# google-deepmind/dqn_zoo

Measured on NVIDIA H100. Metric: learner_grad_steps_per_sec, higher is better.
Workload: dtype f32 (f64 sum tree)

## Files before the change

### dqn_zoo_b200/csrc/dz_async.cuh

```cuda
#pragma once
#include <cuda_runtime.h>
#include <stdint.h>

namespace dz {

__device__ __forceinline__ uint32_t smem_u32(const void* p) { return (uint32_t)__cvta_generic_to_shared(p); }

__device__ __forceinline__ uint32_t smem_pad_1024(const void* base) {
  const uint32_t addr = smem_u32(base);
  return ((addr + 1023u) & ~1023u) - addr;
}

__device__ __forceinline__ void mbar_init(uint64_t* bar, uint32_t count) {
  asm volatile("mbarrier.init.shared::cta.b64 [%0], %1;" ::"r"(smem_u32(bar)), "r"(count));
}
__device__ __forceinline__ void fence_mbarrier_init() { asm volatile("fence.mbarrier_init.release.cluster;" ::: "memory"); }
__device__ __forceinline__ void mbar_arrive(uint64_t* bar) {
  asm volatile("mbarrier.arrive.shared::cta.b64 _, [%0];" ::"r"(smem_u32(bar)) : "memory");
}
__device__ __forceinline__ void mbar_arrive_if(uint64_t* bar, bool pred) {
  asm volatile("{\n.reg .pred p;\nsetp.ne.b32 p, %1, 0;\n@p mbarrier.arrive.shared::cta.b64 _, [%0];\n}\n" ::"r"(smem_u32(bar)),
               "r"((int)pred)
               : "memory");
}
// ... 13 lines not shown
      "r"(parity)
      : "memory");
}

__device__ __forceinline__ bool elect_one() {
  uint32_t pred;
  asm volatile("{\n .reg .pred P;\n elect.sync _|P, 0xffffffff;\n selp.u32 %0, 1, 0, P;\n}\n" : "=r"(pred));
  return pred != 0;
}

__device__ __forceinline__ void bulk_g2s(uint32_t dst_smem, const void* src, uint32_t bytes, uint64_t* bar) {
  asm volatile("cp.async.bulk.shared::cluster.global.mbarrier::complete_tx::bytes [%0], [%1], %2, [%3];" ::"r"(dst_smem),
               "l"(__cvta_generic_to_global(src)), "r"(bytes), "r"(smem_u32(bar))
               : "memory");
}
__device__ __forceinline__ void bulk_s2g(void* dst, const void* src_smem, uint32_t bytes) {
  asm volatile("cp.async.bulk.global.shared::cta.bulk_group [%0], [%1], %2;" ::"l"(__cvta_generic_to_global(dst)),
               "r"(smem_u32(src_smem)), "r"(bytes)
               : "memory");
}
__device__ __forceinline__ void bulk_commit_group() { asm volatile("cp.async.bulk.commit_group;" ::: "memory"); }
__device__ __forceinline__ void bulk_wait_group() { asm volatile("cp.async.bulk.wait_group 0;" ::: "memory"); }
__device__ __forceinline__ void bulk_wait_group_read() { asm volatile("cp.async.bulk.wait_group.read 0;" ::: "memory"); }

__device__ __forceinline__ void tma_load_5d(uint32_t dst_smem, const void* map, uint64_t* bar, int c0, int c1, int c2, int c3, int c4) {
  asm volatile(
      "cp.async.bulk.tensor.5d.shared::cluster.global.mbarrier::complete_tx::bytes [%0], [%1, {%3, %4, %5, %6, %7}], [%2];" ::"r"(dst_smem),
      "l"(reinterpret_cast<uint64_t>(map)), "r"(smem_u32(bar)), "r"(c0), "r"(c1), "r"(c2), "r"(c3), "r"(c4)
      : "memory");
}
__device__ __forceinline__ void prefetch_tensormap(const void* map) {
  asm volatile("prefetch.tensormap [%0];" ::"l"(reinterpret_cast<uint64_t>(map)) : "memory");
}
// ... 5 lines not shown
```

### dqn_zoo_b200/csrc/dz_gemm.cuh

```cuda
#pragma once
#include "dz_common.cuh"

namespace dz {

enum : int { A_PLAIN = 0, A_CONV_F32 = 1, A_CONV_U8 = 2 };

struct FastDiv {
  uint32_t mul, shr;
  int d;
};
inline FastDiv make_fastdiv(int d) {
  FastDiv f;
  f.d = d < 1 ? 1 : d;
  uint32_t s = 0;
  while ((1u << s) < (uint32_t)f.d) ++s;
  f.shr = s;
  f.mul = (uint32_t)((((uint64_t)1 << 32) * (((uint64_t)1 << s) - (uint64_t)f.d)) / (uint64_t)f.d + 1);
  return f;
}
__device__ __forceinline__ int fd_div(int n, const FastDiv& f) {
  return (int)(((uint32_t)__umulhi((uint32_t)n, f.mul) + (uint32_t)n) >> f.shr);
}


// ... 9 lines not shown
  int H, W, Cin, KW, S, OH, OW, seg;
  FastDiv fd_per, fd_ow, fd_seg;
  const float* bias;
  const float* bias2;
  const float* a_scale;
  const float* c_scale;
  const float* mul;
  const float* mask;
  float* Cb;
  float* Cb2;
  int mul_div;
  int relu;
  int bias_shared;
  int splits;
  long long split_stride;
};

constexpr int kMaxProblems = 6;
struct GemmBatch {
  GemmProblem p[kMaxProblems];
  int n;
};

struct ARow {
  const float* f;
  const uint8_t* u;
};

__device__ __forceinline__ ARow a_row_base(const GemmProblem& p, int m) {
  ARow r{nullptr, nullptr};
// ... 350 lines not shown
      if (p.relu) v = fmaxf(v, 0.f);
      p.C[(long long)m * p.ldc + n] = v;
    }
  }
}

template <int BMK, int BN, int BR, int TM, int TN>
__global__ void __launch_bounds__((BMK / TM) * (BN / TN)) gemm_tn_kernel(const __grid_constant__ GemmBatch batch) {
  dz::pdl_enter();
  constexpr int NT = (BMK / TM) * (BN / TN);
  const GemmProblem& p = batch.p[blockIdx.z];
  const int Kext = p.K + ((p.Cb || p.Cb2) ? 1 : 0);
  const int tiles_k = (Kext + BMK - 1) / BMK;
  const int tile_k = blockIdx.y % tiles_k, split = blockIdx.y / tiles_k;
  const int kk0 = tile_k * BMK, n0 = blockIdx.x * BN;
  if (blockIdx.y >= tiles_k * p.splits || n0 >= p.N) return;
  const int rchunks = (p.M + BR - 1) / BR;
  const int per = (rchunks + p.splits - 1) / p.splits;
  const int rc0 = split * per, rc1 = min(rchunks, rc0 + per);

  __shared__ __align__(16) float As[2][BR][BMK + kPad];
  __shared__ __align__(16) float Bs[2][BR][BN + kPad];
  const int tid = threadIdx.x, tx = tid % (BN / TN), ty = tid / (BN / TN);
  constexpr int A_VEC = BR * BMK / 4, B_VEC = BR * BN / 4;
  constexpr int A_PER = (A_VEC + NT - 1) / NT, B_PER = (B_VEC + NT - 1) / NT;
  const bool vecG = (p.ldb % 4 == 0) && ((reinterpret_cast<uintptr_t>(p.B) & 15) == 0);
  Acc<TM, TN> acc;
  acc.clear();
  float4 ra[A_PER], rb[B_PER];
  auto gload = [&](int rc) {
    const int r0 = rc * BR;
// ... 37 lines not shown
      int v = tid + i * NT;
      if (v < B_VEC) *reinterpret_cast<float4*>(&Bs[buf][v / (BN / 4)][(v % (BN / 4)) * 4]) = rb[i];
    }
  };
  if (rc0 < rc1) { gload(rc0); sstore(0); }
  __syncthreads();
  for (int rc = rc0; rc < rc1; ++rc) {
    const int cur = (rc - rc0) & 1;
    const bool more = rc + 1 < rc1;
    if (more) gload(rc + 1);
    tile_fma<BMK, BN, BR, TM, TN, kPad>(As[cur], Bs[cur], ty, tx, acc);
    if (more) sstore(cur ^ 1);
    __syncthreads();
  }

#pragma unroll
  for (int i = 0; i < TM; ++i) {
    int k = kk0 + ty * TM + i;
    if (k >= Kext) continue;
    const int nb = n0 + tx * TN;
    if (TN == 4 && nb + 3 < p.N && (p.N % 4 == 0) && (p.ldc % 4 == 0 || p.split_stride > 0)) {
      float4 v4 = make_float4(acc.v[i][0], acc.v[i][1], acc.v[i][2], acc.v[i][3]);
      if (p.split_stride > 0) {
        *reinterpret_cast<float4*>(p.C + (long long)split * p.split_stride + (long long)k * p.N + nb) = v4;
        continue;
      }
      if (k < p.K) {
        if (p.C) *reinterpret_cast<float4*>(p.C + (long long)k * p.ldc + nb) = v4;
        if (p.C2) {
          float a = p.a_scale[k];
          float4 c = *reinterpret_cast<const float4*>(p.c_scale + nb);
          *reinterpret_cast<float4*>(p.C2 + (long long)k * p.ldc + nb) = make_float4(v4.x * a * c.x, v4.y * a * c.y, v4.z * a * c.z, v4.w * a * c.w);
        }
      } else {
        if (p.Cb) *reinterpret_cast<float4*>(p.Cb + nb) = v4;
        if (p.Cb2) {
          float4 c = *reinterpret_cast<const float4*>(p.c_scale + nb);
          *reinterpret_cast<float4*>(p.Cb2 + nb) = make_float4(v4.x * c.x, v4.y * c.y, v4.z * c.z, v4.w * c.w);
        }
      }
      continue;
    }
#pragma unroll
    for (int j = 0; j < TN; ++j) {
      int n = n0 + tx * TN + j;
      if (n >= p.N) continue;
      float v = acc.v[i][j];
      if (p.split_stride > 0) {
        p.C[(long long)split * p.split_stride + (long long)k * p.N + n] = v;
        continue;
      }
      if (k < p.K) {
        if (p.C) p.C[(long long)k * p.ldc + n] = v;
        if (p.C2) p.C2[(long long)k * p.ldc + n] = v * p.a_scale[k] * p.c_scale[n];
      } else {
        if (p.Cb) p.Cb[n] = v;
        if (p.Cb2) p.Cb2[n] = v * p.c_scale[n];
      }
    }
  }
}

template <int BM, int BNK, int BR, int TM, int TN, bool DUAL>
__global__ void __launch_bounds__((BM / TM) * (BNK / TN)) gemm_nt_kernel(const __grid_constant__ GemmBatch batch) {
  dz::pdl_enter();
  constexpr int NT = (BM / TM) * (BNK / TN);
  const GemmProblem& p = batch.p[blockIdx.z];
  const int tiles_m = (p.M + BM - 1) / BM;
  const int tile_m = blockIdx.y % tiles_m, split = blockIdx.y / tiles_m;
  const int m0 = tile_m * BM, k0 = blockIdx.x * BNK;
  if (blockIdx.y >= tiles_m * p.splits || k0 >= p.K) return;
  const int nchunks = (p.N + BR - 1) / BR;
  const int per = (nchunks + p.splits - 1) / p.splits;
// ... 99 lines not shown
```

### dqn_zoo_b200/csrc/dz_learner.cu

```cuda
#include <algorithm>
#include <cmath>
#include <map>
#include <vector>

#include "dz_async.cuh"
#include "dz_gemm.cuh"
#include "dz_tc.cuh"
#include "dz_internal.cuh"
#include "dz_umma_net.cuh"

namespace dz {


struct TensorInfo {
  std::string name;
  int64_t shape[4];
  int ndim;
  int64_t offset, count;
};

struct Dims {
  int H, W, C;
  int h1, w1, h2, w2, h3, w3;
  int feat;
// ... 292 lines not shown
        int oy = yy / S;
        if (oy >= OH) continue;
        for (int kw = 0; kw < KW; ++kw) {
          int xx = x - kw;
          if (xx < 0 || xx % S) continue;
          int ox = xx / S;
          if (ox >= OW) continue;
          v += dcol[((long long)(b * OH + oy) * OW + ox) * K + (kh * KW + kw) * Cin + c];
        }
      }
    }
    dx[i] = v;
  }
}

__global__ void sum_to_scalar_kernel(const float* __restrict__ v, int n, float* out) {
  dz::pdl_enter();
  __shared__ float s[32];
  float acc = 0.f;
  for (int i = threadIdx.x; i < n; i += blockDim.x) acc += v[i];
  acc = warp_sum(acc);
  if ((threadIdx.x & 31) == 0) s[threadIdx.x >> 5] = acc;
  __syncthreads();
  if (threadIdx.x < 32) {
    acc = threadIdx.x < (blockDim.x >> 5) ? s[threadIdx.x] : 0.f;
    acc = warp_sum(acc);
    if (threadIdx.x == 0) out[0] = acc;
  }
}


constexpr int kSkinnyMaxN = 18;
struct SkinnyHead { const float* A[3]; const float* W[3]; const float* bias[3]; float* out[3]; int M[3]; int n; };

__global__ void __launch_bounds__(256) iqn_head_fwd_kernel(const __grid_constant__ SkinnyHead h, int N) {
  dz::pdl_enter();
  constexpr int K = 512;
  __shared__ __align__(16) float Ws[kSkinnyMaxN * K];
  const int q = blockIdx.y;
  const float* __restrict__ W = h.W[q];
  for (int i = threadIdx.x; i < K * N; i += 256) {
    int k = i / N, n = i - k * N;
// ... 488 lines not shown
      res = e / s;
    } else if (kind == DZ_QRDQN || kind == DZ_IQN) {
      float s = 0.f;
      for (int j = tid; j < nq; j += blockDim.x) s += out[(long long)j * A + a];
      res = block_sum(s, red) / (float)nq;
    } else {
      res = out[a];
    }
    if (tid == 0) q[a] = res;
    __syncthreads();
  }
}


__global__ void __launch_bounds__(256) grad_norm_kernel(const float* __restrict__ g, long long n, float* partials,
                                                        unsigned int* ticket, float* norm_out, int64_t* counters, float* user_norm,
                                                        int sumsq_only) {
  dz::pdl_enter();
  __shared__ float s[32];
  __shared__ bool last;
  float acc = 0.f;
  const long long n4 = n >> 2;
  const float4* g4 = reinterpret_cast<const float4*>(g);
  for (long long i = blockIdx.x * (long long)blockDim.x + threadIdx.x; i < n4; i += (long long)gridDim.x * blockDim.x) {
    float4 v = g4[i];
    acc = fmaf(v.x, v.x, acc); acc = fmaf(v.y, v.y, acc); acc = fmaf(v.z, v.z, acc); acc = fmaf(v.w, v.w, acc);
  }
  acc = warp_sum(acc);
  if ((threadIdx.x & 31) == 0) s[threadIdx.x >> 5] = acc;
  __syncthreads();
  if (threadIdx.x == 0) {
    float t = 0.f;
// ... 3 lines not shown
    unsigned int done = atomicAdd(ticket, 1u);
    last = (done == gridDim.x - 1);
  }
  __syncthreads();
  if (last) {
    __threadfence();
    float t = 0.f;
    for (unsigned int i = threadIdx.x; i < gridDim.x; i += blockDim.x) t += ((volatile float*)partials)[i];
    t = warp_sum(t);
    __syncthreads();
    if ((threadIdx.x & 31) == 0) s[threadIdx.x >> 5] = t;
    __syncthreads();
    if (threadIdx.x == 0) {
      float tot = 0.f;
      for (int i = 0; i < (blockDim.x >> 5); ++i) tot += s[i];
      norm_out[0] = sumsq_only ? tot : sqrtf(tot);
      if (user_norm && !sumsq_only) user_norm[0] = norm_out[0];
      *ticket = 0;
      counters[0] += 1;
    }
  }
}

struct OptArgs {
  int kind; float lr, eps, decay, b1, b2, max_norm;
  float* p; const float* g; float* m; float* v; long long n; const float* norm; const int64_t* counters;
  const float* parts; int nparts; const float* fc_sumsq; float* norm_out; float* user_norm;
  int stages;
};

__device__ __forceinline__ float split_norm(const float* __restrict__ parts, int nparts, const float* __restrict__ fc_sumsq) {
  __shared__ float s_red[8];
  float t = 0.f;
  if (threadIdx.x < 256) {
    for (int i = threadIdx.x; i < nparts; i += 256) t += __ldcg(parts + i);
    t = warp_sum(t);
    if ((threadIdx.x & 31) == 0) s_red[threadIdx.x >> 5] = t;
  }
  __syncthreads();
  float tot = __ldcg(fc_sumsq);
#pragma unroll
  for (int i = 0; i < 8; ++i) tot += s_red[i];
  return sqrtf(tot);
}

__global__ void __launch_bounds__(256) norm_finalize_kernel(const float* parts, int nparts, const float* fc_sumsq, float* norm_out,
                                                            float* user_norm) {
  dz::pdl_enter();
  const float norm = split_norm(parts, nparts, fc_sumsq);
  if (threadIdx.x == 0) { norm_out[0] = norm; if (user_norm) user_norm[0] = norm; }
}

template <int KIND>
__device__ __forceinline__ float opt_one(const OptArgs& o, float p, float g, float& m, float& v, bool clip, float norm,
                                         float inv_c1, float inv_c2) {
  if (clip) g = (g / norm) * o.max_norm;
  float upd;
  if (KIND == DZ_ADAM) {
    float mu = o.b1 * m + (1.0f - o.b1) * g;
    float nu = o.b2 * v + (1.0f - o.b2) * g * g;
    if (fabsf(mu) < 1.17549435e-38f) mu = 0.f;
    if (nu < 1.17549435e-38f) nu = 0.f;
    m = mu; v = nu;
    upd = (mu * inv_c1) / (sqrtf(nu * inv_c2) + o.eps);
  } else {
// ... 20 lines not shown
  const int kOptStages = o.stages;
  uint64_t* full = reinterpret_cast<uint64_t*>(opt_sm + kOptStages * kOptStageBytes);
  const int tid = threadIdx.x;
  const long long n4 = o.n >> 2;
  const long long nchunks = (n4 + kOptChunk - 1) / kOptChunk;
  const long long mine = blockIdx.x < nchunks ? (nchunks - blockIdx.x + gridDim.x - 1) / gridDim.x : 0;
  float4* p4 = reinterpret_cast<float4*>(o.p);
  const float4* g4 = reinterpret_cast<const float4*>(o.g);
  float4* m4 = reinterpret_cast<float4*>(o.m);
  float4* v4 = reinterpret_cast<float4*>(o.v);
  if (tid == 0) {
    for (int s = 0; s < kOptStages; ++s) mbar_init(&full[s], 1);
    fence_mbarrier_init();
  }
  __syncthreads();
  dz::pdl_enter();
  auto issue = [&](long long it, int s) {
    const long long c = blockIdx.x + it * gridDim.x;
    const long long q0 = c * kOptChunk;
    const uint32_t bytes = (uint32_t)(min((long long)kOptChunk, n4 - q0) * 16);
    const uint32_t st = smem_u32(opt_sm + s * kOptStageBytes);
    mbar_expect_tx(&full[s], 4 * bytes);
    bulk_g2s(st, p4 + q0, bytes, &full[s]);
    bulk_g2s(st + kOptChunk * 16, g4 + q0, bytes, &full[s]);
    bulk_g2s(st + 2 * kOptChunk * 16, m4 + q0, bytes, &full[s]);
    bulk_g2s(st + 3 * kOptChunk * 16, v4 + q0, bytes, &full[s]);
  };
  if (tid == 0)
    for (long long it = 0; it < mine && it < kOptStages; ++it) issue(it, (int)it);
  float norm;
  if (o.parts != nullptr) {
    norm = split_norm(o.parts, o.nparts, o.fc_sumsq);
    if (blockIdx.x == 0 && tid == 0) { o.norm_out[0] = norm; if (o.user_norm) o.user_norm[0] = norm; }
  } else {
    norm = o.norm[0];
  }
  const bool clip = o.max_norm > 0.f && !(norm < o.max_norm);
  float c1 = 1.f, c2 = 1.f;
  if (KIND == DZ_ADAM) {
    float t = (float)o.counters[0];
    c1 = 1.0f / (1.0f - powf(o.b1, t));
    c2 = 1.0f / (1.0f - powf(o.b2, t));
  }
  int s = 0;
  uint32_t phase = 0;
  for (long long it = 0; it < mine; ++it) {
    const long long q0 = (blockIdx.x + it * gridDim.x) * (long long)kOptChunk;
    const int valid = (int)min((long long)kOptChunk, n4 - q0);
    float4* sp = reinterpret_cast<float4*>(opt_sm + s * kOptStageBytes);
    float4* sg = sp + kOptChunk;
    float4* smm = sp + 2 * kOptChunk;
    float4* sv = sp + 3 * kOptChunk;
    if (tid == 0 && it > 0) {
      const long long next = it - 1 + kOptStages;
      if (next < mine) {
        bulk_wait_group_read();
        issue(next, s == 0 ? kOptStages - 1 : s - 1);
      }
    }
    mbar_wait(&full[s], phase);
    if (tid < 2 * valid) {
      float2 p = reinterpret_cast<float2*>(sp)[tid], g = reinterpret_cast<float2*>(sg)[tid];
      float2 m = reinterpret_cast<float2*>(smm)[tid], v = reinterpret_cast<float2*>(sv)[tid];
      p.x = opt_one<KIND>(o, p.x, g.x, m.x, v.x, clip, norm, c1, c2);
      p.y = opt_one<KIND>(o, p.y, g.y, m.y, v.y, clip, norm, c1, c2);
      reinterpret_cast<float2*>(sp)[tid] = p; reinterpret_cast<float2*>(smm)[tid] = m; reinterpret_cast<float2*>(sv)[tid] = v;
    }
    fence_proxy_async_shared();
    __syncthreads();
    if (tid == 0) {
      const uint32_t bytes = (uint32_t)valid * 16;
      bulk_s2g(p4 + q0, sp, bytes);
      bulk_s2g(m4 + q0, smm, bytes);
      bulk_s2g(v4 + q0, sv, bytes);
      bulk_commit_group();
    }
    if (++s == kOptStages) { s = 0; phase ^= 1u; }
  }
  if (tid == 0) bulk_wait_group();
}

using OptKernel = void (*)(OptArgs);
OptKernel optimizer_kernel_for(int kind) {
  return kind == DZ_ADAM ? optimizer_bulk_kernel<DZ_ADAM> : optimizer_bulk_kernel<DZ_RMSPROP_CENTERED>;
}

__global__ void act_select_kernel(const float* __restrict__ q, int A, int E, const float* __restrict__ explore, float eps,
                                  int32_t* __restrict__ actions) {
  dz::pdl_enter();
  const int e = blockIdx.x * blockDim.x + threadIdx.x;
  if (e >= E) return;
  int best = 0;
  float bq = q[(long long)e * A];
  for (int a = 1; a < A; ++a) {
// ... 87 lines not shown
  bool opt_smem_set = false;
};

namespace {

constexpr int kNormBlocks = kNumSMs * 4;

int pick_splits(int64_t tiles, int nkb, int max_splits) {
  int best = 1;
  int64_t best_cost = -1;
  for (int s = 1; s <= max_splits; ++s) {
    int64_t cost = ceil_div(tiles * s, kNumSMs) * (ceil_div(nkb, s) + 6);
    if (best_cost < 0 || cost < best_cost) { best_cost = cost; best = s; }
  }
  return best;
}

UmNetDesc make_um_desc(const dz_learner* l);

int64_t carve(dz_learner* l, char* base) {
  const dz_learner_config& c = l->cfg;
  const Dims& d = l->d;
  const int B = c.batch;
  Bump w{base};
  const bool rb = c.kind == DZ_RAINBOW, iqn = c.kind == DZ_IQN;
  int nh[3] = {1, 1, 1};
  if (iqn) { nh[0] = c.tau_samples_s_tm1; nh[1] = c.tau_samples_policy; nh[2] = c.tau_samples_s_t; }
  for (int p = 0; p < 3; ++p) l->n_head[p] = nh[p];
  for (int p = 0; p < 3; ++p) {
    l->act1[p] = w.take<float>((int64_t)B * d.h1 * d.w1 * 32);
// ... 66 lines not shown
    int64_t fwd_rows = (int64_t)B * (nh[0] + nh[1] + nh[2]);
    l->pk_fwd_partial = w.take<float>((int64_t)l->pk_fwd_splits * fwd_rows * 512);
    l->pk_wgrad_partial = w.take<float>((int64_t)l->pk_wgrad_splits * (d.feat + 1) * 512);
  }
  l->loss_terms = w.take<float>(B);
  l->scalars = w.take<float>(8 + kNormBlocks + d.out + 64);
  l->ticket = w.take<unsigned int>(4);
  l->rows_sample[0] = w.take<const uint8_t*>(B);
  l->rows_sample[1] = w.take<const uint8_t*>(B);
  l->rows_act = w.take<const uint8_t*>(B > 4 ? B : 4);
  l->s_a = w.take<int32_t>(B);
  l->s_r = w.take<float>(B);
  l->s_d = w.take<float>(B);
  l->s_w = w.take<float>(B);
  l->q_scratch = w.take<float>(64);
  l->norm_parts = w.take<float>(1024);
  l->um_ws = nullptr;
  UmNetDesc ud = make_um_desc(l);
  if (um_net_supported(ud)) {
    int64_t bytes = um_net_workspace_bytes(ud);
    l->um_ws = w.take<char>(bytes);
    if (!base) l->um_ws = reinterpret_cast<char*>(1);
  }
  return w.used;
}

struct NoiseLayout {
  int64_t stride;
  int64_t a1i, a1o, a2i, a2o, v1i, v1o, v2i, v2o;
};
NoiseLayout noise_layout(const dz_learner_config& c, const Dims& d) {
// ... 77 lines not shown
  }
  if (maxM <= 32) {
    dim3 grid((unsigned)ceil_div(maxN, 64), (unsigned)(ceil_div(maxM, 32) * maxS), gb.n);
    if (dual) return launch_batch(tag, gemm_nn_kernel<32, 64, 16, 2, 4, true>, gb, grid, 256, stream);
    return launch_batch(tag, gemm_nn_kernel<32, 64, 16, 2, 4, false>, gb, grid, 256, stream);
  }
  if (maxN <= 32 && !dual) {
    dim3 grid(1, (unsigned)(ceil_div(maxM, 64) * maxS), gb.n);
    return launch_batch(tag, gemm_nn_kernel<64, 32, 16, 4, 4, false>, gb, grid, 128, stream);
  }
  dim3 grid((unsigned)ceil_div(maxN, 64), (unsigned)(ceil_div(maxM, 64) * maxS), gb.n);
  if (dual) return launch_batch(tag, gemm_nn_kernel<64, 64, 16, 4, 4, true>, gb, grid, 256, stream);
  return launch_batch(tag, gemm_nn_kernel<64, 64, 16, 4, 4, false>, gb, grid, 256, stream);
}

int run_tn(const char* tag, GemmBatch& gb, void* stream) {
  int maxK = 0, maxN = 0, maxS = 1;
  for (int i = 0; i < gb.n; ++i) {
    int kext = gb.p[i].K + ((gb.p[i].Cb || gb.p[i].Cb2) ? 1 : 0);
    maxK = kext > maxK ? kext : maxK;
    maxN = gb.p[i].N > maxN ? gb.p[i].N : maxN;
    maxS = gb.p[i].splits > maxS ? gb.p[i].splits : maxS;
  }
  if (maxN <= 32) {
    dim3 grid(1, (unsigned)(ceil_div(maxK, 64) * maxS), gb.n);
    return launch_batch(tag, gemm_tn_kernel<64, 32, 16, 4, 2>, gb, grid, 256, stream);
  }
  dim3 grid((unsigned)ceil_div(maxN, 64), (unsigned)(ceil_div(maxK, 64) * maxS), gb.n);
  return launch_batch(tag, gemm_tn_kernel<64, 64, 16, 4, 4>, gb, grid, 256, stream);
}

int run_nt(const char* tag, GemmBatch& gb, bool dual, void* stream) {
  int maxM = 0, maxK = 0, maxS = 1;
  for (int i = 0; i < gb.n; ++i) {
    maxM = gb.p[i].M > maxM ? gb.p[i].M : maxM;
    maxK = gb.p[i].K > maxK ? gb.p[i].K : maxK;
    maxS = gb.p[i].splits > maxS ? gb.p[i].splits : maxS;
  }
  if (maxM <= 32) {
    dim3 grid((unsigned)ceil_div(maxK, 64), (unsigned)(ceil_div(maxM, 32) * maxS), gb.n);
    if (dual) return launch_batch(tag, gemm_nt_kernel<32, 64, 16, 2, 4, true>, gb, grid, 256, stream);
    return launch_batch(tag, gemm_nt_kernel<32, 64, 16, 2, 4, false>, gb, grid, 256, stream);
  }
// ... 361 lines not shown
  FinishNTBatch fb;
  memset(&fb, 0, sizeof(fb));
  long long total = 0;
  for (int j = 0; j < njobs; ++j) { fb.f[j] = jobs[j]; total = std::max(total, (long long)jobs[j].M * jobs[j].K); }
  dim3 grid((unsigned)std::min<long long>(ceil_div(total, 256), kNumSMs * 8), (unsigned)njobs);
  DZ_LAUNCH(finish_nt_kernel, grid, 256, 0, stream, fb);
  return DZ_OK;
}
int finish_nt(const GemmProblem* probs, int nsrc, const float* mask, float* out, bool dual, void* stream) {
  FinishNT f = make_finish_nt(probs, nsrc, mask, out, dual);
  return finish_nt_batch(&f, 1, stream);
}

bool split_norm_active(const dz_learner* l);

int backward_torso(dz_learner* l, const uint8_t* const* rows0, void* stream) {
  const Dims& d = l->d;
  const ParamOffsets& o = l->po;
  const int B = l->B;
  float* G = l->buf.d_grads;
  const float* P = l->buf.d_online;
  FinishTNBatch fb;
  fb.n = 0;
  GemmBatch gb;
  if (l->um && l->cfg.kind == DZ_IQN) DZ_TRY(um_split_dact3(l->um, stream));
  float* norm_parts = split_norm_active(l) ? l->norm_parts : nullptr;
  if (l->um) {
    void* ws = l->side3.fork(stream, stream);
    DZ_TRY(um_wgrad_conv3(l->um, ws));
    DZ_TRY(um_wgrad_finish_layer(l->um, 3, G + o.conv_w[2], G + o.conv_b[2], norm_parts, ws));
// ... 66 lines not shown
    fb.f[fb.n++] = FinishTN{p.C, splits, p.split_stride, p.K, 32, G + o.conv_w[0], nullptr, p.Cb, nullptr, nullptr, nullptr};
  }
  void* ws = l->side.tail(stream);
  dim3 grid((unsigned)ceil_div(577 * 64, 256), fb.n);
  DZ_LAUNCH(finish_tn_kernel, grid, 256, 0, ws, fb);
  return l->side.join(stream);
}

int backward_plain(dz_learner* l, void* stream) {
  const Dims& d = l->d;
  const ParamOffsets& o = l->po;
  const int B = l->B;
  float* G = l->buf.d_grads;
  const float* P = l->buf.d_online;
  const bool shared = l->cfg.kind == DZ_DOUBLE_Q || l->cfg.kind == DZ_PRIORITIZED;
  GemmBatch gb;
  gb.n = 1;
  {
    GemmProblem p = zero_problem();
    p.a_mode = A_PLAIN; p.A = l->h1[0][0]; p.lda = 512; p.M = B; p.K = 512;
    p.B = l->dout; p.N = d.out; p.ldb = d.out; p.ldc = d.out;
    p.C = G + o.w2[0]; p.Cb = shared ? l->scalars + 8 + kNormBlocks : G + o.b2[0];
    gb.p[0] = p;
    DZ_TRY(run_tn("head_wgrad", gb, l->side.fork(stream, stream)));
    if (shared) DZ_LAUNCH(sum_to_scalar_kernel, 1, 128, 0, l->side.tail(stream), l->scalars + 8 + kNormBlocks, d.out, G + o.b2[0]);
  }
  bool dh1_split_done = false;
  {
    GemmProblem p = zero_problem();
    p.A = l->dout; p.lda = d.out; p.M = B; p.N = d.out; p.K = 512;
    p.B = P + o.w2[0]; p.ldb = d.out; p.C = l->dh1[0]; p.ldc = 512; p.mask = l->h1[0][0];
    const int splits = d.out > 64 ? (int)std::min<int64_t>(16, ceil_div(d.out, 96)) : 1;
    if (splits > 1) {
      p.splits = splits; p.split_stride = (long long)B * 512; p.C = l->nt_partial; p.mask = nullptr;
      gb.p[0] = p;
      DZ_TRY(run_nt("head_dgrad", gb, false, stream));
      FinishNT job = make_finish_nt(&gb.p[0], 1, l->h1[0][0], l->dh1[0], false, l->um ? um_dh1_hi(l->um, 0) : nullptr,
                                    l->um ? um_dh1_lo(l->um, 0) : nullptr);
      DZ_TRY(finish_nt_batch(&job, 1, stream));
      dh1_split_done = l->um != nullptr;
    } else {
      gb.p[0] = p;
      DZ_TRY(run_nt("head_dgrad", gb, false, stream));
    }
  }
  {
    GemmProblem p = zero_problem();
    p.a_mode = A_PLAIN; p.A = l->act3[0]; p.lda = d.feat; p.M = B; p.K = d.feat;
    p.B = l->dh1[0]; p.N = 512; p.ldb = 512; p.ldc = 512;
    p.C = G + o.w1[0]; p.Cb = G + o.b1[0];
    gb.p[0] = p;
    DZ_TRY(run_tn("fc1_wgrad", gb, l->side.fork(stream, stream)));
  }
  if (l->um) {
    if (!dh1_split_done) DZ_TRY(um_split_dh1(l->um, stream));
    DZ_TRY(um_backward_fc(l->um, nullptr, stream));
  } else {
    GemmProblem p = zero_problem();
    p.A = l->dh1[0]; p.lda = 512; p.M = B; p.N = 512; p.K = d.feat;
    p.B = P + o.w1[0]; p.ldb = 512; p.ldc = d.feat;
    p.splits = l->nt_splits; p.split_stride = (long long)B * d.feat; p.C = l->nt_partial;
    gb.p[0] = p;
    DZ_TRY(run_nt("fc1_dgrad", gb, false, stream));
    DZ_TRY(finish_nt(gb.p, 1, l->act3[0], l->dact3, false, stream));
  }
  return DZ_OK;
}

int backward_rainbow(dz_learner* l, const float* noise, void* stream) {
  const Dims& d = l->d;
  const ParamOffsets& o = l->po;
  const dz_learner_config& c = l->cfg;
  const int B = l->B;
  float* G = l->buf.d_grads;
  const float* P = l->buf.d_online;
  NoiseVecs nz = noise_of(c, d, noise, 0);
  GemmBatch gb;
  gb.n = 2;
  for (int s = 0; s < 2; ++s) {
    int n_out = s == 0 ? c.num_actions * c.num_atoms : c.num_atoms;
    GemmProblem p = zero_problem();
    p.a_mode = A_PLAIN; p.A = l->h1[0][s]; p.lda = 512; p.M = B; p.K = 512;
    p.B = s == 0 ? l->dout : l->doutv; p.N = n_out; p.ldb = n_out; p.ldc = n_out;
    p.C = G + o.w2[s]; p.C2 = G + o.sw2[s]; p.Cb = nullptr; p.Cb2 = G + o.sb2[s];
    p.a_scale = s == 0 ? nz.a2i : nz.v2i; p.c_scale = s == 0 ? nz.a2o : nz.v2o;
    gb.p[s] = p;
  }
  DZ_TRY(run_tn("noisy2_wgrad", gb, l->side.fork(stream, stream)));
  for (int s = 0; s < 2; ++s) {
    int n_out = s == 0 ? c.num_actions * c.num_atoms : c.num_atoms;
    GemmProblem p = zero_problem();
    p.A = s == 0 ? l->dout : l->doutv; p.lda = n_out; p.M = B; p.N = n_out; p.K = 512;
    p.B = P + o.w2[s]; p.B2 = P + o.sw2[s]; p.ldb = n_out;
    p.a_scale = s == 0 ? nz.a2i : nz.v2i; p.c_scale = s == 0 ? nz.a2o : nz.v2o;
    p.ldc = 512;
    p.splits = 4; p.split_stride = (long long)2 * B * 512;
    p.C = l->nt_partial + (long long)s * 4 * p.split_stride;
    gb.p[s] = p;
  }
  DZ_TRY(run_nt("noisy2_dgrad", gb, true, stream));
  {
    FinishNT jobs[2];
    for (int s = 0; s < 2; ++s)
      jobs[s] = make_finish_nt(&gb.p[s], 1, l->h1[0][s], l->dh1[s], true, l->um ? um_dh1_hi(l->um, s) : nullptr,
                               l->um ? um_dh1_lo(l->um, s) : nullptr);
    DZ_TRY(finish_nt_batch(jobs, 2, stream));
  }
  for (int s = 0; s < 2; ++s) {
    GemmProblem p = zero_problem();
    p.a_mode = A_PLAIN; p.A = l->act3[0]; p.lda = d.feat; p.M = B; p.K = d.feat;
    p.B = l->dh1[s]; p.N = 512; p.ldb = 512; p.ldc = 512;
    p.C = G + o.w1[s]; p.C2 = G + o.sw1[s]; p.Cb = G + o.b1[s]; p.Cb2 = G + o.sb1[s];
    p.a_scale = s == 0 ? nz.a1i : nz.v1i; p.c_scale = s == 0 ? nz.a1o : nz.v1o;
    gb.p[s] = p;
  }
  DZ_TRY(run_tn("noisy1_wgrad", gb, l->side.fork(stream, stream)));
  if (l->um) {
    DZ_TRY(um_backward_fc(l->um, noise, stream));
    return DZ_OK;
  }
  for (int s = 0; s < 2; ++s) {
    GemmProblem p = zero_problem();
    p.A = l->dh1[s]; p.lda = 512; p.M = B; p.N = 512; p.K = d.feat;
    p.B = P + o.w1[s]; p.B2 = P + o.sw1[s]; p.ldb = 512;
    p.a_scale = s == 0 ? nz.a1i : nz.v1i; p.c_scale = s == 0 ? nz.a1o : nz.v1o;
    p.ldc = d.feat;
    p.splits = l->nt_splits; p.split_stride = (long long)2 * B * d.feat;
    p.C = l->nt_partial + (long long)s * l->nt_splits * p.split_stride;
    gb.p[s] = p;
  }
  DZ_TRY(run_nt("noisy1_dgrad", gb, true, stream));
// ... 112 lines not shown
      p.splits = splits; p.split_stride = (long long)(c.latent_dim + 1) * d.feat; p.C = part_embed;
      gb.p[0] = p;
      DZ_TRY(run_tn("iqn_embed_wgrad", gb, l->side.fork(stream, stream)));
      fb.f[fb.n++] = FinishTN{p.C, splits, p.split_stride, c.latent_dim, d.feat, G + o.embed_w, nullptr, p.Cb, nullptr, nullptr, nullptr};
    }
  }
  long long mx = 0;
  for (int q = 0; q < fb.n; ++q) mx = std::max<long long>(mx, (long long)(fb.f[q].K + 1) * fb.f[q].N);
  dim3 grid((unsigned)std::min<long long>(ceil_div(mx, 256), kNumSMs * 8), fb.n);
  DZ_LAUNCH(finish_tn_kernel, grid, 256, 0, l->side.tail(stream), fb);
  return DZ_OK;
}

bool split_norm_active(const dz_learner* l) { return l->um != nullptr && l->cfg.kind != DZ_IQN; }

int norm_fc_range(dz_learner* l, bool apply, void* stream) {
  const long long begin = l->po.fc_begin;
  const long long n = l->lay.total - begin;
  DZ_LAUNCH(grad_norm_kernel, kNormBlocks, 256, 0, stream, l->buf.d_grads + begin, n, l->scalars + 8, l->ticket, l->scalars + 1,
            apply ? l->buf.d_counters : l->buf.d_counters + 3, (float*)nullptr, 1);
  return DZ_OK;
}

int run_optimizer(dz_learner* l, float* user_norm, bool apply, void* stream) {
  const dz_learner_config& c = l->cfg;
  long long n = l->lay.total;
  float* norm = l->scalars;
  const bool split = split_norm_active(l);
  const float* parts = split ? l->norm_parts : nullptr;
  const int nparts = split ? um_norm_slots(l->um) : 0;
  if (!split) {
    DZ_LAUNCH(grad_norm_kernel, kNormBlocks, 256, 0, stream, l->buf.d_grads, n, l->scalars + 8, l->ticket, norm,
              apply ? l->buf.d_counters : l->buf.d_counters + 3, user_norm, 0);
  } else if (!apply) {
    DZ_LAUNCH(norm_finalize_kernel, 1, 256, 0, stream, parts, nparts, l->scalars + 1, norm, user_norm);
  }
  if (!apply) return DZ_OK;
  OptArgs o{c.optimizer, c.learning_rate, c.opt_eps, c.rms_decay, c.adam_b1, c.adam_b2, c.max_global_grad_norm,
            l->buf.d_online, l->buf.d_grads, l->buf.d_opt_state, l->buf.d_opt_state + n, n, norm, l->buf.d_counters,
            parts, nparts, l->scalars + 1, norm, user_norm};
  o.stages = kOptRingStages;
  const OptKernel kernel = optimizer_kernel_for(c.optimizer);
  if (!l->opt_smem_set) {
    DZ_CUDA_OK(cudaFuncSetAttribute(kernel, cudaFuncAttributeMaxDynamicSharedMemorySize, kOptSmem));
    l->opt_smem_set = true;
  }
  const long long nchunks = ((o.n >> 2) + kOptChunk - 1) / kOptChunk;
  const unsigned grid = (unsigned)std::max<long long>(1, std::min<long long>((long long)kNumSMs * kOptBlocksPerSM, nchunks));
  DZ_LAUNCH_NAMED("optimizer_kernel", kernel, grid, kOptThreads, kOptSmem, stream, o);
  return DZ_OK;
}

struct WriteBack { const dz_replay_view* view; const int64_t* indices; const float* priorities; double alpha; };

int update_impl(dz_learner* l, const dz_batch* batch, const dz_update_outputs* out, int apply_update, float* max_seen,
// ... 63 lines not shown
  } else {
    if (c.kind == DZ_QRDQN) { L.N = c.num_quantiles; L.Ksel = c.num_quantiles; L.Nt = c.num_quantiles; }
    else { L.N = c.tau_samples_s_tm1; L.Ksel = c.tau_samples_policy; L.Nt = c.tau_samples_s_t; }
    size_t smem = (32 + c.num_actions + L.Nt + 2 * L.N) * sizeof(float);
    DZ_LAUNCH(loss_quantile_kernel, B, 256, smem, stream, L);
  }
  {
    void* ls = l->side.fork(stream, stream);
    DZ_LAUNCH(loss_mean_kernel, 1, 32, 0, ls, l->loss_terms, B, out->d_loss, max_seen, L.priorities);
    if (wb) DZ_TRY(launch_update_priorities(wb->view, wb->indices, wb->priorities, B, wb->alpha, wb->view->capacity, ls));
  }

  if (c.kind == DZ_RAINBOW) DZ_TRY(backward_rainbow(l, batch->d_noise, stream));
  else if (c.kind == DZ_IQN) DZ_TRY(backward_iqn(l, stream));
  else DZ_TRY(backward_plain(l, stream));
  if (split_norm_active(l)) {
    DZ_TRY(norm_fc_range(l, apply_update != 0, l->side.tail(stream)));
  }
  DZ_TRY(backward_torso(l, batch->d_s_tm1_rows, stream));

  DZ_TRY(l->side2.join(stream));
  DZ_TRY(l->side.join(stream));
  DZ_TRY(run_optimizer(l, out->d_grad_norm, apply_update != 0, stream));
  return DZ_OK;
}

}


extern "C" {

int dz_learner_plan_query(const dz_learner_config* cfg, dz_learner_plan* out) {
  DZ_TRY(validate(*cfg));
// ... 560 lines not shown
int dz_test_learner_buffer(dz_learner* l, const char* name, float** d_ptr, int64_t* count) {
  const std::string n = name;
  const int64_t rows0 = (int64_t)l->B * l->n_head[0];
  if (n == "act3") { *d_ptr = l->act3[0]; *count = (int64_t)l->B * l->d.feat; }
  else if (n == "act1") { *d_ptr = l->act1[0]; *count = (int64_t)l->B * l->d.h1 * l->d.w1 * 32; }
  else if (n == "act2") { *d_ptr = l->act2[0]; *count = (int64_t)l->B * l->d.h2 * l->d.w2 * 64; }
  else if (n == "h1_val") { *d_ptr = l->h1[0][1]; *count = l->h1[0][1] ? rows0 * 512 : 0; }
  else if (n == "iqn_e0") { *d_ptr = l->E0; *count = l->E0 ? rows0 * l->d.feat : 0; }
  else if (n == "h1") { *d_ptr = l->h1[0][0]; *count = rows0 * 512; }
  else if (n == "dh1") { *d_ptr = l->dh1[0]; *count = rows0 * 512; }
  else if (n == "iqn_hi") {
    if (l->pk_on) return fail(DZ_EINVAL, "iqn_hi is not materialised on the packed tensor-core path");
    *d_ptr = l->hi[0]; *count = l->hi[0] ? rows0 * l->d.feat : 0;
  }
  else if (n == "iqn_dhi") { *d_ptr = l->dhi; *count = l->dhi ? rows0 * l->d.feat : 0; }
  else return fail(DZ_EINVAL, "unknown buffer '%s'", name);
  if (!*d_ptr) return fail(DZ_EINVAL, "buffer '%s' is not used by this agent kind", name);
  return DZ_OK;
}

}
```

Measured before the change: 3109.

## Fuse FC grad-norm partials into wgrad epilogues and prefetch optimizer state before PDL wait

After: 3170 (median of 6 runs). +2.0%, better.

```diff
diff --git a/dqn_zoo_b200/csrc/dz_async.cuh b/dqn_zoo_b200/csrc/dz_async.cuh
--- a/dqn_zoo_b200/csrc/dz_async.cuh
+++ b/dqn_zoo_b200/csrc/dz_async.cuh
@@ -51,9 +51,19 @@
                "l"(__cvta_generic_to_global(src)), "r"(bytes), "r"(smem_u32(bar))
                : "memory");
 }
-__device__ __forceinline__ void bulk_s2g(void* dst, const void* src_smem, uint32_t bytes) {
-  asm volatile("cp.async.bulk.global.shared::cta.bulk_group [%0], [%1], %2;" ::"l"(__cvta_generic_to_global(dst)),
-               "r"(smem_u32(src_smem)), "r"(bytes)
+__device__ __forceinline__ uint64_t l2_evict_first_policy() {
+  uint64_t p;
+  asm volatile("createpolicy.fractional.L2::evict_first.b64 %0, 1.0;" : "=l"(p));
+  return p;
+}
+__device__ __forceinline__ void bulk_g2s_hint(uint32_t dst_smem, const void* src, uint32_t bytes, uint64_t* bar, uint64_t policy) {
+  asm volatile("cp.async.bulk.shared::cluster.global.mbarrier::complete_tx::bytes.L2::cache_hint [%0], [%1], %2, [%3], %4;"
+               ::"r"(dst_smem), "l"(__cvta_generic_to_global(src)), "r"(bytes), "r"(smem_u32(bar)), "l"(policy)
+               : "memory");
+}
+__device__ __forceinline__ void bulk_s2g_hint(void* dst, const void* src_smem, uint32_t bytes, uint64_t policy) {
+  asm volatile("cp.async.bulk.global.shared::cta.bulk_group.L2::cache_hint [%0], [%1], %2, %3;"
+               ::"l"(__cvta_generic_to_global(dst)), "r"(smem_u32(src_smem)), "r"(bytes), "l"(policy)
                : "memory");
 }
 __device__ __forceinline__ void bulk_commit_group() { asm volatile("cp.async.bulk.commit_group;" ::: "memory"); }
diff --git a/dqn_zoo_b200/csrc/dz_gemm.cuh b/dqn_zoo_b200/csrc/dz_gemm.cuh
--- a/dqn_zoo_b200/csrc/dz_gemm.cuh
+++ b/dqn_zoo_b200/csrc/dz_gemm.cuh
@@ -47,6 +47,7 @@
   int bias_shared;
   int splits;
   long long split_stride;
+  float* norm_part;
 };
 
 constexpr int kMaxProblems = 6;
@@ -427,7 +428,11 @@
   const int tiles_k = (Kext + BMK - 1) / BMK;
   const int tile_k = blockIdx.y % tiles_k, split = blockIdx.y / tiles_k;
   const int kk0 = tile_k * BMK, n0 = blockIdx.x * BN;
-  if (blockIdx.y >= tiles_k * p.splits || n0 >= p.N) return;
+  float* const norm_slot = p.norm_part ? p.norm_part + blockIdx.y * gridDim.x + blockIdx.x : nullptr;
+  if (blockIdx.y >= tiles_k * p.splits || n0 >= p.N) {
+    if (norm_slot && threadIdx.x == 0) *norm_slot = 0.f;
+    return;
+  }
   const int rchunks = (p.M + BR - 1) / BR;
   const int per = (rchunks + p.splits - 1) / p.splits;
   const int rc0 = split * per, rc1 = min(rchunks, rc0 + per);
@@ -495,6 +500,8 @@
     __syncthreads();
   }
 
+  float sq = 0.f;
+  auto sq4 = [&](const float4& x) { sq = fmaf(x.x, x.x, sq); sq = fmaf(x.y, x.y, sq); sq = fmaf(x.z, x.z, sq); sq = fmaf(x.w, x.w, sq); };
 #pragma unroll
   for (int i = 0; i < TM; ++i) {
     int k = kk0 + ty * TM + i;
@@ -507,17 +514,21 @@
         continue;
       }
       if (k < p.K) {
-        if (p.C) *reinterpret_cast<float4*>(p.C + (long long)k * p.ldc + nb) = v4;
+        if (p.C) { *reinterpret_cast<float4*>(p.C + (long long)k * p.ldc + nb) = v4; sq4(v4); }
         if (p.C2) {
           float a = p.a_scale[k];
           float4 c = *reinterpret_cast<const float4*>(p.c_scale + nb);
-          *reinterpret_cast<float4*>(p.C2 + (long long)k * p.ldc + nb) = make_float4(v4.x * a * c.x, v4.y * a * c.y, v4.z * a * c.z, v4.w * a * c.w);
+          const float4 w = make_float4(v4.x * a * c.x, v4.y * a * c.y, v4.z * a * c.z, v4.w * a * c.w);
+          *reinterpret_cast<float4*>(p.C2 + (long long)k * p.ldc + nb) = w;
+          sq4(w);
         }
       } else {
-        if (p.Cb) *reinterpret_cast<float4*>(p.Cb + nb) = v4;
+        if (p.Cb) { *reinterpret_cast<float4*>(p.Cb + nb) = v4; if (!p.bias_shared) sq4(v4); }
         if (p.Cb2) {
           float4 c = *reinterpret_cast<const float4*>(p.c_scale + nb);
-          *reinterpret_cast<float4*>(p.Cb2 + nb) = make_float4(v4.x * c.x, v4.y * c.y, v4.z * c.z, v4.w * c.w);
+          const float4 w = make_float4(v4.x * c.x, v4.y * c.y, v4.z * c.z, v4.w * c.w);
+          *reinterpret_cast<float4*>(p.Cb2 + nb) = w;
+          sq4(w);
         }
       }
       continue;
@@ -532,12 +543,24 @@
         continue;
       }
       if (k < p.K) {
-        if (p.C) p.C[(long long)k * p.ldc + n] = v;
-        if (p.C2) p.C2[(long long)k * p.ldc + n] = v * p.a_scale[k] * p.c_scale[n];
+        if (p.C) { p.C[(long long)k * p.ldc + n] = v; sq = fmaf(v, v, sq); }
+        if (p.C2) { const float w = v * p.a_scale[k] * p.c_scale[n]; p.C2[(long long)k * p.ldc + n] = w; sq = fmaf(w, w, sq); }
       } else {
-        if (p.Cb) p.Cb[n] = v;
-        if (p.Cb2) p.Cb2[n] = v * p.c_scale[n];
-      }
+        if (p.Cb) { p.Cb[n] = v; if (!p.bias_shared) sq = fmaf(v, v, sq); }
+        if (p.Cb2) { const float w = v * p.c_scale[n]; p.Cb2[n] = w; sq = fmaf(w, w, sq); }
+      }
+    }
+  }
+  if (norm_slot) {
+    __shared__ float s_sq[NT / 32];
+    sq = warp_sum(sq);
+    if ((tid & 31) == 0) s_sq[tid >> 5] = sq;
+    __syncthreads();
+    if (tid == 0) {
+      float t = 0.f;
+#pragma unroll
+      for (int w = 0; w < NT / 32; ++w) t += s_sq[w];
+      *norm_slot = t;
     }
   }
 }
diff --git a/dqn_zoo_b200/csrc/dz_learner.cu b/dqn_zoo_b200/csrc/dz_learner.cu
--- a/dqn_zoo_b200/csrc/dz_learner.cu
+++ b/dqn_zoo_b200/csrc/dz_learner.cu
@@ -330,7 +330,7 @@
   }
 }
 
-__global__ void sum_to_scalar_kernel(const float* __restrict__ v, int n, float* out) {
+__global__ void sum_to_scalar_kernel(const float* __restrict__ v, int n, float* out, float* sq_out) {
   dz::pdl_enter();
   __shared__ float s[32];
   float acc = 0.f;
@@ -341,7 +341,7 @@
   if (threadIdx.x < 32) {
     acc = threadIdx.x < (blockDim.x >> 5) ? s[threadIdx.x] : 0.f;
     acc = warp_sum(acc);
-    if (threadIdx.x == 0) out[0] = acc;
+    if (threadIdx.x == 0) { out[0] = acc; if (sq_out) sq_out[0] = acc * acc; }
   }
 }
 
@@ -860,8 +860,7 @@
 
 
 __global__ void __launch_bounds__(256) grad_norm_kernel(const float* __restrict__ g, long long n, float* partials,
-                                                        unsigned int* ticket, float* norm_out, int64_t* counters, float* user_norm,
-                                                        int sumsq_only) {
+                                                        unsigned int* ticket, float* norm_out, int64_t* counters, float* user_norm) {
   dz::pdl_enter();
   __shared__ float s[32];
   __shared__ bool last;
@@ -895,8 +894,8 @@
     if (threadIdx.x == 0) {
       float tot = 0.f;
       for (int i = 0; i < (blockDim.x >> 5); ++i) tot += s[i];
-      norm_out[0] = sumsq_only ? tot : sqrtf(tot);
-      if (user_norm && !sumsq_only) user_norm[0] = norm_out[0];
+      norm_out[0] = sqrtf(tot);
+      if (user_norm) user_norm[0] = norm_out[0];
       *ticket = 0;
       counters[0] += 1;
     }
@@ -905,31 +904,37 @@
 
 struct OptArgs {
   int kind; float lr, eps, decay, b1, b2, max_norm;
-  float* p; const float* g; float* m; float* v; long long n; const float* norm; const int64_t* counters;
-  const float* parts; int nparts; const float* fc_sumsq; float* norm_out; float* user_norm;
+  float* p; const float* g; float* m; float* v; long long n; const float* norm; int64_t* counters;
+  const float* parts; int nparts; float* norm_out; float* user_norm; unsigned int* ticket;
   int stages;
 };
 
-__device__ __forceinline__ float split_norm(const float* __restrict__ parts, int nparts, const float* __restrict__ fc_sumsq) {
+__device__ __forceinline__ float split_norm(const float* __restrict__ parts, int nparts) {
   __shared__ float s_red[8];
   float t = 0.f;
   if (threadIdx.x < 256) {
-    for (int i = threadIdx.x; i < nparts; i += 256) t += __ldcg(parts + i);
+    for (int i0 = threadIdx.x; i0 < nparts; i0 += 8 * 256) {
+      float x[8];
+#pragma unroll
+      for (int j = 0; j < 8; ++j) x[j] = i0 + j * 256 < nparts ? __ldcg(parts + i0 + j * 256) : 0.f;
+#pragma unroll
+      for (int j = 0; j < 8; ++j) t += x[j];
+    }
     t = warp_sum(t);
     if ((threadIdx.x & 31) == 0) s_red[threadIdx.x >> 5] = t;
   }
   __syncthreads();
-  float tot = __ldcg(fc_sumsq);
+  float tot = 0.f;
 #pragma unroll
   for (int i = 0; i < 8; ++i) tot += s_red[i];
   return sqrtf(tot);
 }
 
-__global__ void __launch_bounds__(256) norm_finalize_kernel(const float* parts, int nparts, const float* fc_sumsq, float* norm_out,
-                                                            float* user_norm) {
+__global__ void __launch_bounds__(256) norm_finalize_kernel(const float* parts, int nparts, float* norm_out, float* user_norm,
+                                                            int64_t* counter) {
   dz::pdl_enter();
-  const float norm = split_norm(parts, nparts, fc_sumsq);
-  if (threadIdx.x == 0) { norm_out[0] = norm; if (user_norm) user_norm[0] = norm; }
+  const float norm = split_norm(parts, nparts);
+  if (threadIdx.x == 0) { norm_out[0] = norm; if (user_norm) user_norm[0] = norm; counter[0] += 1; }
 }
 
 template <int KIND>
@@ -980,23 +985,29 @@
     fence_mbarrier_init();
   }
   __syncthreads();
-  dz::pdl_enter();
-  auto issue = [&](long long it, int s) {
+  const uint64_t once = l2_evict_first_policy();
+  auto issue = [&](long long it, int s, bool pmv, bool grad) {
     const long long c = blockIdx.x + it * gridDim.x;
     const long long q0 = c * kOptChunk;
     const uint32_t bytes = (uint32_t)(min((long long)kOptChunk, n4 - q0) * 16);
     const uint32_t st = smem_u32(opt_sm + s * kOptStageBytes);
-    mbar_expect_tx(&full[s], 4 * bytes);
-    bulk_g2s(st, p4 + q0, bytes, &full[s]);
-    bulk_g2s(st + kOptChunk * 16, g4 + q0, bytes, &full[s]);
-    bulk_g2s(st + 2 * kOptChunk * 16, m4 + q0, bytes, &full[s]);
-    bulk_g2s(st + 3 * kOptChunk * 16, v4 + q0, bytes, &full[s]);
+    if (pmv) {
+      mbar_expect_tx(&full[s], 4 * bytes);
+      bulk_g2s_hint(st, p4 + q0, bytes, &full[s], once);
+      bulk_g2s_hint(st + 2 * kOptChunk * 16, m4 + q0, bytes, &full[s], once);
+      bulk_g2s_hint(st + 3 * kOptChunk * 16, v4 + q0, bytes, &full[s], once);
+    }
+    if (grad) bulk_g2s(st + kOptChunk * 16, g4 + q0, bytes, &full[s]);
   };
   if (tid == 0)
-    for (long long it = 0; it < mine && it < kOptStages; ++it) issue(it, (int)it);
+    for (long long it = 0; it < mine && it < kOptStages; ++it) issue(it, (int)it, true, false);
+  dz::pdl_enter();
+  if (tid == 0)
+    for (long long it = 0; it < mine && it < kOptStages; ++it) issue(it, (int)it, false, true);
   float norm;
+  const int64_t count = o.counters[0] + (o.parts != nullptr ? 1 : 0);
   if (o.parts != nullptr) {
-    norm = split_norm(o.parts, o.nparts, o.fc_sumsq);
+    norm = split_norm(o.parts, o.nparts);
     if (blockIdx.x == 0 && tid == 0) { o.norm_out[0] = norm; if (o.user_norm) o.user_norm[0] = norm; }
   } else {
     norm = o.norm[0];
@@ -1004,7 +1015,7 @@
   const bool clip = o.max_norm > 0.f && !(norm < o.max_norm);
   float c1 = 1.f, c2 = 1.f;
   if (KIND == DZ_ADAM) {
-    float t = (float)o.counters[0];
+    float t = (float)count;
     c1 = 1.0f / (1.0f - powf(o.b1, t));
     c2 = 1.0f / (1.0f - powf(o.b2, t));
   }
@@ -1021,7 +1032,7 @@
       const long long next = it - 1 + kOptStages;
       if (next < mine) {
         bulk_wait_group_read();
-        issue(next, s == 0 ? kOptStages - 1 : s - 1);
+        issue(next, s == 0 ? kOptStages - 1 : s - 1, true, true);
       }
     }
     mbar_wait(&full[s], phase);
@@ -1036,14 +1047,20 @@
     __syncthreads();
     if (tid == 0) {
       const uint32_t bytes = (uint32_t)valid * 16;
-      bulk_s2g(p4 + q0, sp, bytes);
-      bulk_s2g(m4 + q0, smm, bytes);
-      bulk_s2g(v4 + q0, sv, bytes);
+      bulk_s2g_hint(p4 + q0, sp, bytes, once);
+      bulk_s2g_hint(m4 + q0, smm, bytes, once);
+      bulk_s2g_hint(v4 + q0, sv, bytes, once);
       bulk_commit_group();
     }
     if (++s == kOptStages) { s = 0; phase ^= 1u; }
   }
-  if (tid == 0) bulk_wait_group();
+  if (tid == 0) {
+    bulk_wait_group();
+    if (o.parts != nullptr) {
+      __threadfence();
+      if (atomicAdd(o.ticket, 1u) == gridDim.x - 1) { o.counters[0] = count; *o.ticket = 0; }
+    }
+  }
 }
 
 using OptKernel = void (*)(OptArgs);
@@ -1161,6 +1178,18 @@
     if (best_cost < 0 || cost < best_cost) { best_cost = cost; best = s; }
   }
   return best;
+}
+
+dim3 tn_grid(int maxKext, int maxN, int maxS, int nprob) {
+  return dim3(maxN <= 32 ? 1u : (unsigned)ceil_div(maxN, 64), (unsigned)(ceil_div(maxKext, 64) * maxS), (unsigned)nprob);
+}
+
+int fc_norm_slots(const dz_learner_config& c, const Dims& d) {
+  auto ctas = [](dim3 g) { return (int)(g.x * g.y * g.z); };
+  if (c.kind == DZ_IQN) return 0;
+  const int nstream = c.kind == DZ_RAINBOW ? 2 : 1;
+  const int shared = c.kind == DZ_DOUBLE_Q || c.kind == DZ_PRIORITIZED ? 1 : 0;
+  return ctas(tn_grid(512 + 1, d.out, 1, nstream)) + shared + ctas(tn_grid(d.feat + 1, 512, 1, nstream));
 }
 
 UmNetDesc make_um_desc(const dz_learner* l);
@@ -1257,7 +1286,7 @@
   l->s_d = w.take<float>(B);
   l->s_w = w.take<float>(B);
   l->q_scratch = w.take<float>(64);
-  l->norm_parts = w.take<float>(1024);
+  l->norm_parts = w.take<float>(um_norm_slots(nullptr) + fc_norm_slots(c, d));
   l->um_ws = nullptr;
   UmNetDesc ud = make_um_desc(l);
   if (um_net_supported(ud)) {
@@ -1365,7 +1394,7 @@
   return launch_batch(tag, gemm_nn_kernel<64, 64, 16, 4, 4, false>, gb, grid, 256, stream);
 }
 
-int run_tn(const char* tag, GemmBatch& gb, void* stream) {
+int run_tn(const char* tag, GemmBatch& gb, void* stream, float** norm_cursor = nullptr) {
   int maxK = 0, maxN = 0, maxS = 1;
   for (int i = 0; i < gb.n; ++i) {
     int kext = gb.p[i].K + ((gb.p[i].Cb || gb.p[i].Cb2) ? 1 : 0);
@@ -1373,11 +1402,15 @@
     maxN = gb.p[i].N > maxN ? gb.p[i].N : maxN;
     maxS = gb.p[i].splits > maxS ? gb.p[i].splits : maxS;
   }
-  if (maxN <= 32) {
-    dim3 grid(1, (unsigned)(ceil_div(maxK, 64) * maxS), gb.n);
-    return launch_batch(tag, gemm_tn_kernel<64, 32, 16, 4, 2>, gb, grid, 256, stream);
-  }
-  dim3 grid((unsigned)ceil_div(maxN, 64), (unsigned)(ceil_div(maxK, 64) * maxS), gb.n);
+  const dim3 grid = tn_grid(maxK, maxN, maxS, gb.n);
+  if (norm_cursor && *norm_cursor) {
+    for (int i = 0; i < gb.n; ++i) {
+      if (gb.p[i].split_stride > 0) return fail(DZ_EINVAL, "run_tn: split-norm slots need the non-partial epilogue");
+      gb.p[i].norm_part = *norm_cursor;
+      *norm_cursor += grid.x * grid.y;
+    }
+  }
+  if (maxN <= 32) return launch_batch(tag, gemm_tn_kernel<64, 32, 16, 4, 2>, gb, grid, 256, stream);
   return launch_batch(tag, gemm_tn_kernel<64, 64, 16, 4, 4>, gb, grid, 256, stream);
 }
 
@@ -1769,6 +1802,13 @@
 
 bool split_norm_active(const dz_learner* l);
 
+float* fc_norm_base(dz_learner* l) { return split_norm_active(l) ? l->norm_parts + um_norm_slots(l->um) : nullptr; }
+int check_fc_norm_slots(const dz_learner* l, const float* end) {
+  if (end && end != l->norm_parts + um_norm_slots(l->um) + fc_norm_slots(l->cfg, l->d))
+    return fail(DZ_EINVAL, "FC weight gradients: split-norm slot count differs from fc_norm_slots");
+  return DZ_OK;
+}
+
 int backward_torso(dz_learner* l, const uint8_t* const* rows0, void* stream) {
   const Dims& d = l->d;
   const ParamOffsets& o = l->po;
@@ -1865,16 +1905,20 @@
   float* G = l->buf.d_grads;
   const float* P = l->buf.d_online;
   const bool shared = l->cfg.kind == DZ_DOUBLE_Q || l->cfg.kind == DZ_PRIORITIZED;
+  float* slot = fc_norm_base(l);
   GemmBatch gb;
   gb.n = 1;
   {
     GemmProblem p = zero_problem();
     p.a_mode = A_PLAIN; p.A = l->h1[0][0]; p.lda = 512; p.M = B; p.K = 512;
     p.B = l->dout; p.N = d.out; p.ldb = d.out; p.ldc = d.out;
-    p.C = G + o.w2[0]; p.Cb = shared ? l->scalars + 8 + kNormBlocks : G + o.b2[0];
+    p.C = G + o.w2[0]; p.Cb = shared ? l->scalars + 8 + kNormBlocks : G + o.b2[0]; p.bias_shared = shared ? 1 : 0;
     gb.p[0] = p;
-    DZ_TRY(run_tn("head_wgrad", gb, l->side.fork(stream, stream)));
-    if (shared) DZ_LAUNCH(sum_to_scalar_kernel, 1, 128, 0, l->side.tail(stream), l->scalars + 8 + kNormBlocks, d.out, G + o.b2[0]);
+    DZ_TRY(run_tn("head_wgrad", gb, l->side.fork(stream, stream), &slot));
+    if (shared) {
+      DZ_LAUNCH(sum_to_scalar_kernel, 1, 128, 0, l->side.tail(stream), l->scalars + 8 + kNormBlocks, d.out, G + o.b2[0], slot);
+      if (slot) ++slot;
+    }
   }
   bool dh1_split_done = false;
   {
@@ -1901,8 +1945,9 @@
     p.B = l->dh1[0]; p.N = 512; p.ldb = 512; p.ldc = 512;
     p.C = G + o.w1[0]; p.Cb = G + o.b1[0];
     gb.p[0] = p;
-    DZ_TRY(run_tn("fc1_wgrad", gb, l->side.fork(stream, stream)));
-  }
+    DZ_TRY(run_tn("fc1_wgrad", gb, l->side.fork(stream, stream), &slot));
+  }
+  DZ_TRY(check_fc_norm_slots(l, slot));
   if (l->um) {
     if (!dh1_split_done) DZ_TRY(um_split_dh1(l->um, stream));
     DZ_TRY(um_backward_fc(l->um, nullptr, stream));
@@ -1926,6 +1971,7 @@
   float* G = l->buf.d_grads;
   const float* P = l->buf.d_online;
   NoiseVecs nz = noise_of(c, d, noise, 0);
+  float* slot = fc_norm_base(l);
   GemmBatch gb;
   gb.n = 2;
   for (int s = 0; s < 2; ++s) {
@@ -1937,7 +1983,7 @@
     p.a_scale = s == 0 ? nz.a2i : nz.v2i; p.c_scale = s == 0 ? nz.a2o : nz.v2o;
     gb.p[s] = p;
   }
-  DZ_TRY(run_tn("noisy2_wgrad", gb, l->side.fork(stream, stream)));
+  DZ_TRY(run_tn("noisy2_wgrad", gb, l->side.fork(stream, stream), &slot));
   for (int s = 0; s < 2; ++s) {
     int n_out = s == 0 ? c.num_actions * c.num_atoms : c.num_atoms;
     GemmProblem p = zero_problem();
@@ -1965,7 +2011,8 @@
     p.a_scale = s == 0 ? nz.a1i : nz.v1i; p.c_scale = s == 0 ? nz.a1o : nz.v1o;
     gb.p[s] = p;
   }
-  DZ_TRY(run_tn("noisy1_wgrad", gb, l->side.fork(stream, stream)));
+  DZ_TRY(run_tn("noisy1_wgrad", gb, l->side.fork(stream, stream), &slot));
+  DZ_TRY(check_fc_norm_slots(l, slot));
   if (l->um) {
     DZ_TRY(um_backward_fc(l->um, noise, stream));
     return DZ_OK;
@@ -2108,31 +2155,23 @@
 
 bool split_norm_active(const dz_learner* l) { return l->um != nullptr && l->cfg.kind != DZ_IQN; }
 
-int norm_fc_range(dz_learner* l, bool apply, void* stream) {
-  const long long begin = l->po.fc_begin;
-  const long long n = l->lay.total - begin;
-  DZ_LAUNCH(grad_norm_kernel, kNormBlocks, 256, 0, stream, l->buf.d_grads + begin, n, l->scalars + 8, l->ticket, l->scalars + 1,
-            apply ? l->buf.d_counters : l->buf.d_counters + 3, (float*)nullptr, 1);
-  return DZ_OK;
-}
-
 int run_optimizer(dz_learner* l, float* user_norm, bool apply, void* stream) {
   const dz_learner_config& c = l->cfg;
   long long n = l->lay.total;
   float* norm = l->scalars;
   const bool split = split_norm_active(l);
   const float* parts = split ? l->norm_parts : nullptr;
-  const int nparts = split ? um_norm_slots(l->um) : 0;
+  const int nparts = split ? um_norm_slots(l->um) + fc_norm_slots(c, l->d) : 0;
   if (!split) {
     DZ_LAUNCH(grad_norm_kernel, kNormBlocks, 256, 0, stream, l->buf.d_grads, n, l->scalars + 8, l->ticket, norm,
-              apply ? l->buf.d_counters : l->buf.d_counters + 3, user_norm, 0);
+              apply ? l->buf.d_counters : l->buf.d_counters + 3, user_norm);
   } else if (!apply) {
-    DZ_LAUNCH(norm_finalize_kernel, 1, 256, 0, stream, parts, nparts, l->scalars + 1, norm, user_norm);
+    DZ_LAUNCH(norm_finalize_kernel, 1, 256, 0, stream, parts, nparts, norm, user_norm, l->buf.d_counters + 3);
   }
   if (!apply) return DZ_OK;
   OptArgs o{c.optimizer, c.learning_rate, c.opt_eps, c.rms_decay, c.adam_b1, c.adam_b2, c.max_global_grad_norm,
             l->buf.d_online, l->buf.d_grads, l->buf.d_opt_state, l->buf.d_opt_state + n, n, norm, l->buf.d_counters,
-            parts, nparts, l->scalars + 1, norm, user_norm};
+            parts, nparts, norm, user_norm, l->ticket + 1};
   o.stages = kOptRingStages;
   const OptKernel kernel = optimizer_kernel_for(c.optimizer);
   if (!l->opt_smem_set) {
@@ -2226,9 +2265,6 @@
   if (c.kind == DZ_RAINBOW) DZ_TRY(backward_rainbow(l, batch->d_noise, stream));
   else if (c.kind == DZ_IQN) DZ_TRY(backward_iqn(l, stream));
   else DZ_TRY(backward_plain(l, stream));
-  if (split_norm_active(l)) {
-    DZ_TRY(norm_fc_range(l, apply_update != 0, l->side.tail(stream)));
-  }
   DZ_TRY(backward_torso(l, batch->d_s_tm1_rows, stream));
 
   DZ_TRY(l->side2.join(stream));
@@ -2819,6 +2855,10 @@
     *d_ptr = l->hi[0]; *count = l->hi[0] ? rows0 * l->d.feat : 0;
   }
   else if (n == "iqn_dhi") { *d_ptr = l->dhi; *count = l->dhi ? rows0 * l->d.feat : 0; }
+  else if (n == "norm_parts") {
+    if (!split_norm_active(l)) return fail(DZ_EINVAL, "norm_parts: this learner takes its norm in one kernel");
+    *d_ptr = l->norm_parts; *count = um_norm_slots(l->um) + fc_norm_slots(l->cfg, l->d);
+  }
   else return fail(DZ_EINVAL, "unknown buffer '%s'", name);
   if (!*d_ptr) return fail(DZ_EINVAL, "buffer '%s' is not used by this agent kind", name);
   return DZ_OK;
```
